# AlexIoannides/bodywork-mlops-demo

Hardware: NVIDIA H100
Metric: train rows/sec (N x 128 least-squares fit) (higher is better)
Workload: dtype bf16x2 (hi+lo) MMA operands, f32 accumulate, f64 fold+solve

## Files before the change

### bodywork-mlops-demo_b200/csrc/b2_internal.cuh

```cuda
#pragma once
#include <cuda.h>
#include <cuda_bf16.h>
#include <cuda_runtime.h>
#include <stdint.h>
#include <stdio.h>
#include <string.h>

#include <type_traits>

#include "../../include/b2gram.h"

namespace b2 {

constexpr int kMaxD = B2_MAX_D;
constexpr int kMaxS = kMaxD + 2;
constexpr int kKernelEventPairs = 64;
constexpr int kMaxRanks = 8;
constexpr size_t kXchgSlotDoubles = (size_t)kMaxS * kMaxS;
constexpr size_t kXchgDataDoubles = 2 * kMaxRanks * kXchgSlotDoubles;
constexpr size_t kXchgBytes = kXchgDataDoubles * sizeof(double) + 256;

constexpr int kTcRows = 64;
constexpr int kTcM = 128;
constexpr int kTcEMax = 16;
// ... 15 lines not shown
constexpr int kRfB0 = kMaxD;
constexpr int kRfMean = kMaxD + 1;
constexpr int kRfPrevBeta = 2 * kMaxD + 1;
constexpr int kRfPrevB0 = 3 * kMaxD + 1;
constexpr int kRfStep = 3 * kMaxD + 2;
constexpr int kRfGrad = 3 * kMaxD + 3;
constexpr int kRfDoubles = kRfGrad + kGradOut;
constexpr int kOutRefineStep = 2 * kMaxD + 3;
constexpr int kOutRefineGuard = 2 * kMaxD + 4;

constexpr int kMaxAlphas = B2_MAX_ALPHAS;
constexpr int kLooQ = 0;
constexpr int kLooLam = kMaxD * kMaxD;
constexpr int kLooMean = kLooLam + kMaxD;
constexpr int kLooC = kLooMean + kMaxD;
constexpr int kLooMisc = kLooC + kMaxD;
constexpr int kLooAlpha = kLooMisc + 8;
constexpr int kLooCw = kLooAlpha + kMaxAlphas;
constexpr int kLooW = kLooCw + kMaxD * kMaxAlphas;
constexpr int kLooSum = kLooW + kMaxD * kMaxAlphas;
constexpr int kLooDoubles = kLooSum + kMaxAlphas;

struct EnetArgs {
  double l1_ratio, eps, tol;
  int n_alphas, grid, max_iter, positive, fit_intercept;
  double* alphas;
  const double* coef_init;
  double *coefs, *intercepts, *gaps, *iters, *tol_out;
  const double* folds = nullptr;
  const double* l1_ratios = nullptr;
  int n_folds = 1, n_l1 = 1;
  double* mse = nullptr;
};

constexpr int kByCoef = 0;
constexpr int kByMisc = kMaxD;
constexpr int kByLambda = kMaxD + 8;
constexpr int kBySigma = 2 * kMaxD + 8;
constexpr int kByDoubles = kBySigma + kMaxD * kMaxD;
constexpr int kStdSigma = 0;
constexpr int kStdMean = kMaxD * kMaxD;
constexpr int kStdCoef = kStdMean + kMaxD;
constexpr int kStdMisc = kStdCoef + kMaxD;
constexpr int kStdDoubles = kStdMisc + 8;
struct BayesArgs {
  double a1, a2, l1, l2, alpha_init, lambda_init;
  double threshold_lambda, tol;
  int max_iter, compute_score, fit_intercept;
  const double* anchor;
  double *out, *scores, *A;
};

constexpr int kGlmSteps = 21;
constexpr int kGlmGrad = 8;
constexpr int kGlmHess = 144;
constexpr int kGlmHp = 144;
constexpr int kGlmPart = kGlmHess + kGlmHp * kGlmHp;
constexpr int kGlmOp = kGlmPart;
constexpr int kGlmOpW = 0, kGlmOpStep = kMaxD, kGlmOpMisc = 2 * kMaxD;
constexpr int kGlmDoubles = kGlmOp + 2 * kMaxD + 8;
enum GlmMode { kGlmGradient = 0, kGlmHessian = 1, kGlmLadder = 2 };
enum GlmFamily { kGlmTweedie = 0, kGlmBinomial = 1 };
constexpr int kGlmCorrect = 7;
enum LabelWord { kLabelKept = 0, kLabelNonFinite, kLabelNonIntegral, kLabelMin, kLabelMax, kLabelNMin, kLabelNMax,
                 kLabelWords };

constexpr int kMaxFolds = 254;
int launch_fold_ranges(b2_ctx* ctx, const uint8_t* fold_of_row, int64_t n, int n_folds, unsigned long long* range);
int launch_fold_sum(b2_ctx* ctx, const double* folds, int n_folds, int d, double* S);

inline int narrow_dp(int d) { return d <= 1 ? 1 : d <= 2 ? 2 : d <= 4 ? 4 : d <= 8 ? 8 : 16; }

void set_error(const char* fmt, ...);

#define B2_CUDA(call)                                                                      \
  do {                                                                                     \
    cudaError_t e_ = (call);                                                               \
    if (e_ != cudaSuccess) {                                                               \
      b2::set_error("%s failed: %s (%s:%d)", #call, cudaGetErrorString(e_), __FILE__, __LINE__); \
      return B2_E_CUDA;                                                                    \
    }                                                                                      \
  } while (0)

}

struct b2_ctx {
  int device = 0;
  int sm_count = 0;
  size_t hbm_bytes = 0;
  char name[128] = {0};
  cudaStream_t stream = nullptr;
  cudaStream_t copy_stream = nullptr;
  cudaEvent_t ev_t0 = nullptr, ev_t1 = nullptr;
  cudaEvent_t ev_k[b2::kKernelEventPairs][2];
  int k_pairs = 0;
  int64_t launches = 0;

  int kernel_mode = B2_KERNEL_AUTO;
  int drain_rows = 8192;
  int precision = B2_PRECISION_SPLIT;

  int d = 0;
  double* S = nullptr;

  double* tc_part = nullptr;
  double* tc_red = nullptr;
  float* shift = nullptr;
  bool solve_attr_set = false;
  double* solve_host = nullptr;
  struct TmCache {
    const void* X = nullptr; const float* y = nullptr; const uint8_t* mask = nullptr;
    int64_t n = 0, ldx = 0; int d = 0, x_dtype = -1;
    int y_map_2d = 0, m_map_2d = 0;
    alignas(64) unsigned char tmX[128], tmY[128], tmM[128];
  } tm_cache;
  double* simt_part = nullptr;
  int simt_ctas = 0;
  double* score_part = nullptr;
  int score_ctas = 0;
  double* coef_dev = nullptr;
  double* grad_part = nullptr;
  double* refine = nullptr;
  double* loo = nullptr;
  double* loo_part = nullptr;
  double* enet = nullptr;
  size_t enet_doubles = 0;
  double* folds = nullptr;
  size_t folds_doubles = 0;
  int n_folds = 0;
  int folds_d = 0;
  unsigned long long* fold_range = nullptr;
  double* glm = nullptr;
  double* glm_part = nullptr;
  double* coef_host = nullptr;
  cudaEvent_t ev_coef[2] = {nullptr, nullptr};
  int coef_slot = 0;
  long long* synth_count = nullptr;
  double* solve_out = nullptr;
  void* stage_x[2] = {nullptr, nullptr};
  float* stage_y[2] = {nullptr, nullptr};
  uint8_t* stage_m[2] = {nullptr, nullptr};
  size_t stage_bytes_x = 0;
  int64_t stage_rows = 0;
  cudaEvent_t ev_copied[2] = {nullptr, nullptr};
  cudaEvent_t ev_consumed[2] = {nullptr, nullptr};
  bool ev_consumed_valid[2] = {false, false};
  char* row_out[2] = {nullptr, nullptr};
  size_t row_out_bytes = 0;
  void* bounce[2] = {nullptr, nullptr};
  cudaEvent_t ev_bounce[2] = {nullptr, nullptr};
  bool s_zero_pending = false;
  void* comm = nullptr;
  int n_ranks = 1, rank = 0;
  double* xchg = nullptr;
  double* xchg_peer[8] = {nullptr};
  bool p2p_ready = false;
  bool p2p_local = false;
  unsigned int xchg_epoch = 0;
  unsigned long long xchg_timeout_ns = 10000000000ull;
  bool xchg_pending = false;
  unsigned int* xchg_status_host = nullptr;
  unsigned int* tc_sync = nullptr;
  int fused_fits = 0;
  int sm_limit = 0;
  bool sm_limit_auto = false;
};

namespace b2 {

inline double* score_totals(const b2_ctx* ctx) { return ctx->score_part + (size_t)ctx->score_ctas * kNStats; }

template <typename... P, typename... A>
int launch_smem(void (*kernel)(P...), int grid, int threads, uint32_t smem, cudaStream_t stream, A... args) {
  B2_CUDA(cudaFuncSetAttribute(kernel, cudaFuncAttributeMaxDynamicSharedMemorySize, smem));
  kernel<<<grid, threads, smem, stream>>>(args...);
  B2_CUDA(cudaGetLastError());
  return B2_OK;
}
template <int V, int... Vs, typename F>
int with_int(int v, F&& f) {
  if constexpr (sizeof...(Vs) == 0) return f(std::integral_constant<int, V>{});
  else return v == V ? f(std::integral_constant<int, V>{}) : with_int<Vs...>(v, f);
}
template <typename F>
int with_rows(int x_dtype, const void* X, F&& f) {
  if (x_dtype == B2_F32) return f(static_cast<const float*>(X));
  return f(static_cast<const __nv_bfloat16*>(X));
}
template <typename P>
using row_t = std::remove_const_t<std::remove_pointer_t<P>>;

// ... 88 lines not shown
```

### bodywork-mlops-demo_b200/csrc/gram_shift.cu

```cuda
#include <cuda_bf16.h>

#include "b2_internal.cuh"
#include "b2_ptx.cuh"

namespace b2 {
namespace {

constexpr int kShiftBlocks = 64;
constexpr int kShiftStride = kMaxD + 1;
constexpr int kShiftPartOff = kMaxD + 1;
constexpr int kShiftTicketOff = kShiftPartOff + kShiftBlocks * kShiftStride;

__host__ __device__ __forceinline__ int64_t shift_samples(int64_t n) { return n < 2048 ? n : 2048; }

__device__ __forceinline__ float shift_round(float c, bool round_bf16) {
  return round_bf16 ? __bfloat162float(__float2bfloat16_rn(c)) : c;
}
__device__ __noinline__ float shift_value(const float* sp, int j, bool round_bf16) {
  float acc = 0.f;
  int cnt = 0;
#pragma unroll 8
  for (int b = 0; b < kShiftBlocks; ++b) {
    const float p = sp[b * kShiftStride + j];
    if (p == p) { acc += p; ++cnt; }
  }
  return shift_round(cnt > 0 ? acc / (float)cnt : 0.f, round_bf16);
}

constexpr int kShiftCols = 160;
constexpr int kShiftGroups = 4;

template <typename T>
__global__ void __launch_bounds__(kShiftCols * kShiftGroups)
tc_shift_kernel(const T* __restrict__ X, const float* __restrict__ y, int64_t n, int d, int64_t ldx, float* shift) {
  __shared__ float sub[kShiftGroups][kShiftCols];
  __shared__ int subn[kShiftGroups][kShiftCols];
  __shared__ bool last_block;
  __shared__ float part_s[kShiftBlocks * kShiftStride];
  float* sp = shift + kShiftPartOff;
  const int j = threadIdx.x % kShiftCols, g = threadIdx.x / kShiftCols;
  const int64_t samples = shift_samples(n);
  const int64_t stride = n / samples;
  const int64_t per = (samples + kShiftBlocks - 1) / kShiftBlocks;
  const int64_t s0 = blockIdx.x * per;
  const int64_t s1 = (s0 + per < samples) ? s0 + per : samples;
  float acc = 0.f;
  int cnt = 0;
  if (j <= d) {
#pragma unroll 8
    for (int64_t s = s0 + g; s < s1; s += kShiftGroups) {
      const int64_t row = s * stride;
      const float v = (j < d) ? raw_ld_global<T>(X + row * ldx + j) : __ldg(y + row);
      const bool finite = fabsf(v) <= 3.0e38f;
      acc += finite ? v : 0.f;
      cnt += finite ? 1 : 0;
    }
  }
  sub[g][j] = acc;
  subn[g][j] = cnt;
  __syncthreads();
  if (g == 0 && j <= d) {
    const int c = subn[0][j] + subn[1][j] + subn[2][j] + subn[3][j];
    sp[blockIdx.x * kShiftStride + (j == d ? kMaxD : j)] =
        c > 0 ? (((sub[0][j] + sub[1][j]) + sub[2][j]) + sub[3][j]) / (float)c : __int_as_float(0x7fc00000);
    __threadfence();
  }
  __syncthreads();
  unsigned int* ticket = reinterpret_cast<unsigned int*>(shift + kShiftTicketOff);
  if (threadIdx.x == 0) last_block = atomicAdd(ticket, 1u) == gridDim.x - 1;
  __syncthreads();
  if (!last_block) return;
  __threadfence();
  if (j <= d) {
    const int col = j == d ? kMaxD : j;
    float p[kShiftBlocks / kShiftGroups];
#pragma unroll
    for (int i = 0; i < kShiftBlocks / kShiftGroups; ++i) p[i] = __ldcg(sp + (g + kShiftGroups * i) * kShiftStride + col);
#pragma unroll
    for (int i = 0; i < kShiftBlocks / kShiftGroups; ++i) part_s[(g + kShiftGroups * i) * kShiftStride + col] = p[i];
  }
  __syncthreads();
  for (int k = threadIdx.x; k <= kMaxD; k += blockDim.x)
    shift[k] = k == kMaxD ? shift_value(part_s, kMaxD, false) : (k < d ? shift_value(part_s, k, sizeof(T) == 2) : 0.f);
  if (threadIdx.x == 0) *ticket = 0u;
}

}

size_t gram_shift_bytes() { return sizeof(float) * (kShiftTicketOff + 1); }

int launch_gram_shift(b2_ctx* ctx, const void* X, int x_dtype, const float* y, int64_t n, int d, int64_t ldx) {
  if (x_dtype == B2_F32)
    tc_shift_kernel<float><<<kShiftBlocks, kShiftCols * kShiftGroups, 0, ctx->stream>>>(
        static_cast<const float*>(X), y, n, d, ldx, ctx->shift);
  else
    tc_shift_kernel<__nv_bfloat16><<<kShiftBlocks, kShiftCols * kShiftGroups, 0, ctx->stream>>>(
        static_cast<const __nv_bfloat16*>(X), y, n, d, ldx, ctx->shift);
  B2_CUDA(cudaGetLastError());
  ctx->launches += 1;
  return B2_OK;
}

}
```

### bodywork-mlops-demo_b200/csrc/gram_tc.cu

```cuda
#include <cuda_bf16.h>
#include <stdlib.h>

#include "b2_internal.cuh"
#include "b2_ptx.cuh"
#include "b2_shift.cuh"
#include "b2_xchg.cuh"

namespace b2 {
namespace {

constexpr int kConsumerWGs = 2;
constexpr int kXformWarps = 8;
constexpr int kThreads = 128 * (kConsumerWGs + 2);
constexpr int kFirstXformWarp = 4 * kConsumerWGs;
constexpr int kTmaWarp = kFirstXformWarp;
constexpr int kEWarp = kFirstXformWarp + 1;
static_assert(kFirstXformWarp + kXformWarps == kThreads / 32, "warp roles");
constexpr int kProducers = kXformWarps;
constexpr int kConsumerWarps = 4 * kConsumerWGs;
constexpr int kKGroups = kTcRows / 8;
constexpr uint32_t kRawStageBytes = kTcRows * kMaxD * 4;
constexpr uint32_t kOpSBO = 128;
constexpr uint32_t kOpLBO = (16 + 2 + 16) * kOpSBO;
constexpr uint32_t kOpEOff = 16 * kOpSBO;
// ... 263 lines not shown
  const int dp = d + 2;
  const int a = min(idx / dp, idx % dp), b = max(idx / dp, idx % dp);
  auto P = [&](int acc, int i, int j) { return __ldcg(red + tc_part_index(acc, i, j, ew)); };
  auto s1 = [&](int i) {
    double t = 0.0;
    for (int blk = 0; blk < pack; ++blk) {
      const int r = blk * d + i, e = kTcM + 3 * blk;
      t += d2 ? P(0, r, e) + P(1, r, e) : P(0, r, e);
    }
    return t;
  };
  auto sxy = [&](int i) {
    double t = 0.0;
    for (int blk = 0; blk < pack; ++blk) {
      const int r = blk * d + i, e = kTcM + 3 * blk;
      t += d2 ? P(0, r, e + 1) + P(0, r, e + 2) + P(1, r, e + 1) + P(1, r, e + 2) : P(0, r, e + 1) + P(0, r, e + 2);
    }
    return t;
  };
  auto G = [&](int i, int j) {
    double g = 0.0;
    for (int blk = 0; blk < pack; ++blk) {
      const int ia = blk * d + i, ib = blk * d + j;
      const double g1 = P(0, min(ia, ib), max(ia, ib));
      g += d2 ? g1 + P(1, ia, ib) + P(1, ib, ia) : g1;
    }
    return g;
  };
  return unshift_entry(a, b, d, c, G, s1, sxy, __ldcg(red + kTcAccElems + 2), __ldcg(red + kTcAccElems + 0),
                       __ldcg(red + kTcAccElems + 1));
}

template <typename T, int DFIX, bool SPLIT, bool RAWB = false, int EW = 8>
__global__ void __launch_bounds__(kThreads, 1)
gram_tc_kernel(const __grid_constant__ CUtensorMap tmX, const __grid_constant__ CUtensorMap tmY,
               const __grid_constant__ CUtensorMap tmM, int y_map_2d, int has_mask, int keep,
               int64_t n_rows, int d_arg, int pack, int d_orig, const float* __restrict__ shift,
               int chunk_tiles, double* __restrict__ part, uint32_t wait_ns, uint32_t dbg_arg) {
#ifdef B2_DEV_KNOBS
  const uint32_t dbg = dbg_arg;
#else
  constexpr uint32_t dbg = 0u;
  (void)dbg_arg;
#endif
  using G = TcGeo<RAWB>;
  constexpr int kRawStages = G::kRawStages, kOpStages = G::kOpStages;
  constexpr uint32_t kOffRaw = G::kOffRaw, kOffOp = G::kOffOp, kOffY = G::kOffY, kOffMask = G::kOffMask;
  const int d = DFIX ? DFIX : d_arg;
  extern __shared__ uint8_t smem_raw[];
  const uint32_t sbase = (smem_u32(smem_raw) + 1023u) & ~1023u;
  uint8_t* smem = smem_raw + (sbase - smem_u32(smem_raw));
  const int warp = threadIdx.x >> 5;
  const int lane = threadIdx.x & 31;

  const uint32_t bar_raw_full = sbase + G::kOffBar;
  const uint32_t bar_raw_empty = bar_raw_full + 8 * kRawStages;
  const uint32_t bar_op_full = bar_raw_empty + 8 * kRawStages;
  const uint32_t bar_op_empty = bar_op_full + 8 * kOpStages;
  float* shift_s = reinterpret_cast<float*>(smem + G::kOffShift);

  const int64_t total_tiles = (n_rows + kTcRows - 1) / kTcRows;
  const int64_t tile_begin = (int64_t)blockIdx.x * total_tiles / gridDim.x;
  const int64_t tile_end = (int64_t)(blockIdx.x + 1) * total_tiles / gridDim.x;
  const int my_tiles = (int)(tile_end - tile_begin);

  if (threadIdx.x == 0) {
    for (int s = 0; s < kRawStages; ++s) {
      mbar_init(bar_raw_full + 8 * s, 1);
      mbar_init(bar_raw_empty + 8 * s, kProducers + (RAWB ? kConsumerWarps : 0));
    }
    for (int s = 0; s < kOpStages; ++s) {
      mbar_init(bar_op_full + 8 * s, kProducers);
      mbar_init(bar_op_empty + 8 * s, kConsumerWarps);
    }
    asm volatile("fence.mbarrier_init.release.cluster;" ::: "memory");
  }
  if (warp == kTmaWarp && lane == 0) {
    tma_prefetch_desc(&tmX);
    tma_prefetch_desc(&tmY);
    if (has_mask) tma_prefetch_desc(&tmM);
  }
  for (uint32_t o = threadIdx.x * 16; o < kOpStages * kOpStageBytes; o += kThreads * 16)
    *reinterpret_cast<uint4*>(smem + kOffOp + o) = make_uint4(0, 0, 0, 0);
  for (int j = threadIdx.x; j <= kMaxD; j += kThreads)
    shift_s[j] = j == kMaxD ? shift[kMaxD] : (j < pack * d_orig ? shift[j % d_orig] : 0.f);
  fence_proxy_async_smem();
  __syncthreads();

  if (warp < kConsumerWarps) {
    asm volatile("setmaxnreg.inc.sync.aligned.u32 %0;" ::"n"(G::kConsumerRegs));
    auto consume = [&](auto wg_c) {
      constexpr int WG = decltype(wg_c)::value;
      constexpr int kF1 = kTcM - 64 * WG;
      constexpr int kF2 = RAWB ? kF1 : kTcM;
      constexpr int kC1 = 64 * WG;
      constexpr int kR1 = (kF1 + EW) / 2, kR2 = (kF2 + EW) / 2;
      float acc1[kR1], acc2[kR2];
      using H = TcSums<DFIX, SPLIT, RAWB, EW, WG>;
      double* my_part = part + (size_t)blockIdx.x * kTcAccElems;
      double sums[H::kRegs > 0 ? H::kRegs : 1];
      const bool on_chip_off = (dbg & 256u) != 0u;
      auto slab_addr = [&](int s, int ln) {
        return sbase + G::kOffSlab + (uint32_t)(((4 * H::kSlabBase + (warp & 3) * H::kSlab + s) * 32 + ln) * 8);
      };
      auto store = [&](auto n_regs, int dst_acc, int col0, bool add, auto val) {
        const int ln = (int)lane_id(), row0 = 64 * WG + 16 * (warp & 3) + (ln >> 2);
#pragma unroll
        for (int r = 0; r < decltype(n_regs)::value; ++r) {
          const int col = col0 + 8 * (r >> 2) + 2 * (ln & 3) + (r & 1), h = (r >> 1) & 1, i = row0 + 8 * h;
          const bool lower = dst_acc == 0 && col < kTcM && i > col;
          const double v = val(r, col, h);
          const bool on_chip = dst_acc == 0 && r >= H::kFirstSlab;
          if (on_chip && r >= H::kFirstReg) {
            double& s = sums[r - H::kFirstReg];
            s = add ? __dadd_rn(s, v) : v;
          } else if (on_chip) {
            const uint32_t a = slab_addr(r - H::kFirstSlab, ln);
            st_shared_f64_if(a, add ? __dadd_rn(ld_shared_f64(a), v) : v, !on_chip_off);
          }
          put_f64(my_part + tc_part_index(dst_acc, i, col, EW), v, add, !lower && (!on_chip || on_chip_off));
        }
      };
      auto flush = [&]() {
        const int ln = (int)lane_id(), row0 = 64 * WG + 16 * (warp & 3) + (ln >> 2);
#pragma unroll
        for (int r = H::kFirstSlab; r < H::kR1; ++r) {
          const int col = kC1 + 8 * (r >> 2) + 2 * (ln & 3) + (r & 1), i = row0 + 8 * ((r >> 1) & 1);
          const double s = r >= H::kFirstReg ? sums[r - H::kFirstReg] : ld_shared_f64(slab_addr(r - H::kFirstSlab, ln));
          put_f64(my_part + tc_part_index(0, i, col, EW), s, false, !(col < kTcM && i > col) && !on_chip_off);
        }
      };
      auto drain = [&](const auto& acc, int dst_acc, int col0, bool add) {
        constexpr int kR = sizeof(acc) / sizeof(float);
        if constexpr (RAWB) {
          constexpr int kF = 2 * kR - EW;
          const double s1[2] = {(double)__shfl_sync(0xffffffffu, acc[kF / 2], lane & ~3),
                                (double)__shfl_sync(0xffffffffu, acc[kF / 2 + 2], lane & ~3)};
          store(std::integral_constant<int, kR>{}, dst_acc, col0, add, [&](int r, int col, int h) {
            return col < kTcM ? (double)acc[r] - (double)shift_s[col] * s1[h] : (double)acc[r];
          });
        } else {
          store(std::integral_constant<int, kR>{}, dst_acc, col0, add, [&](int r, int, int) { return (double)acc[r]; });
        }
      };
      auto release = [&](int tile) {
        mbar_arrive(bar_op_empty + 8 * (tile % kOpStages));
        if constexpr (RAWB) mbar_arrive(bar_raw_empty + 8 * (tile % kRawStages));
      };
      constexpr uint32_t a_off = (uint32_t)WG * 8 * kOpSBO;
      int os = 0, held = -1, in_chunk = 0;
      uint32_t oph = 0;
      bool first_chunk = true;
      for (int it = 0; it < my_tiles; ++it) {
        mbar_wait(bar_op_full + 8 * os, oph, wait_ns);
        const uint32_t op_addr = sbase + kOffOp + os * kOpStageBytes;
        wgmma_fence();
#pragma unroll
        for (int k2 = 0; k2 < kTcRows / 16; ++k2) {
          const uint32_t k_addr = op_addr + k2 * 2 * kOpLBO;
          const uint64_t hi_desc = make_smem_desc(k_addr + a_off), lo_desc = make_smem_desc(k_addr + kOpLoOff + a_off);
          const uint32_t sc1 = (in_chunk > 0 || k2 > 0) ? 1u : 0u, sc2 = (it > 0 || k2 > 0) ? 1u : 0u;
          if constexpr (RAWB) {
            const uint64_t x_desc = make_raw_desc(sbase + kOffRaw + (uint32_t)(it % kRawStages) * kRawStageBytes +
                                                  (uint32_t)WG * kRawBoxBytes + k2 * 16 * 128);
            const uint64_t e_desc = make_smem_desc(k_addr + kOpEOff);
            if (!(dbg & 2u)) {
// ... 103 lines not shown
            st_shared_u16(dst + (3 * bl + 2) * 16, yl);
            if (RAWB && has_mask && !use) {
              const uint32_t row = raw_addr + (uint32_t)rr * 128;
              const uint32_t z[4] = {0u, 0u, 0u, 0u};
#pragma unroll
              for (int q = 0; q < 8; ++q) { st_shared_v4(row + 16 * q, z); st_shared_v4(row + kRawBoxBytes + 16 * q, z); }
            }
            a += yv;
            b = fmaf(yv, yv, b);
            c += use ? 1.f : 0.f;
          }
        }
        const uint32_t es = esum();
        st_shared_f64(es, ld_shared_f64(es) + (double)a);
        st_shared_f64(es + 256, ld_shared_f64(es + 256) + (double)b);
        st_shared_f64(es + 512, ld_shared_f64(es + 512) + (double)c);
      }
      if (i < d && !(dbg & 128u)) {
        float c_i[2];
        ld_vals_vec<float, 2>(sbase + G::kOffShift + 4 * (uint32_t)i, c_i);
        for (int g = t / nb; g < kKGroups; g += kXformWarps / nb) {
          const int r0 = g * 8;
          float v0[8], v1[8];
          const uint32_t src = raw_addr + (uint32_t)r0 * ((uint32_t)d * sizeof(T)) + (uint32_t)i * sizeof(T);
#pragma unroll
          for (int k = 0; k < 8; ++k) {
            const uint32_t a = RAWB ? raw_addr + (uint32_t)(i >> 6) * kRawBoxBytes + (uint32_t)(r0 + k) * 128 +
                                          ((((uint32_t)(i & 63) >> 3) ^ (uint32_t)k) << 4) + (uint32_t)(i & 7) * 2
                                    : src + (uint32_t)k * ((uint32_t)d * sizeof(T));
            float x[2];
            if (dbg & 8u) { x[0] = __uint_as_float(src + k); x[1] = __uint_as_float(src - k); }
            else ld_vals_vec<T, 2>(a, x);
            v0[k] = x[0] - c_i[0];
            v1[k] = x[1] - c_i[1];
          }
          if (!full_tile) {
            const int blk = i / d_orig;
#pragma unroll
            for (int k = 0; k < 8; ++k) {
              bool use = (r0 + k) < rows_valid;
              if (use && has_mask) use = (ld_shared_u8(m_addr + (r0 + k) * pack + blk) == (uint32_t)keep);
              if (!use) { v0[k] = 0.f; v1[k] = 0.f; }
            }
          }
          uint32_t h0[4], l0[4], h1[4], l1[4];
#pragma unroll
          for (int p = 0; p < 4; ++p) {
            if constexpr (SPLIT) {
              split2(v0[2 * p], v0[2 * p + 1], h0[p], l0[p]);
              split2(v1[2 * p], v1[2 * p + 1], h1[p], l1[p]);
            } else {
              const __nv_bfloat162 e0 = __floats2bfloat162_rn(v0[2 * p], v0[2 * p + 1]);
              const __nv_bfloat162 e1 = __floats2bfloat162_rn(v1[2 * p], v1[2 * p + 1]);
              h0[p] = *reinterpret_cast<const uint32_t*>(&e0);
              h1[p] = *reinterpret_cast<const uint32_t*>(&e1);
              l0[p] = l1[p] = 0u;
            }
          }
          if (!(dbg & 4u)) {
            const uint32_t dst = op_addr + (uint32_t)g * kOpLBO + st_off;
            uint32_t f[4], s[4];
#pragma unroll
            for (int p = 0; p < 4; ++p) { f[p] = swp ? h1[p] : h0[p]; s[p] = swp ? h0[p] : h1[p]; }
            st_shared_v4(dst + 16 * swp, f);
            st_shared_v4(dst + 16 - 16 * swp, s);
            if constexpr (SPLIT) {
#pragma unroll
              for (int p = 0; p < 4; ++p) { f[p] = swp ? l1[p] : l0[p]; s[p] = swp ? l0[p] : l1[p]; }
              st_shared_v4(dst + kOpLoOff + 16 * swp, f);
              st_shared_v4(dst + kOpLoOff + 16 - 16 * swp, s);
            }
          }
        }
      }
      if (!(dbg & 32u)) fence_proxy_async_smem();
      __syncwarp();
      if (lane == 0) {
        mbar_arrive(bar_op_full + 8 * os);
        mbar_arrive(bar_raw_empty + 8 * rs);
      }
      if (++rs == kRawStages) { rs = 0; rph ^= 1; }
      if (++os == kOpStages) { os = 0; oph ^= 1; }
    }
    if (warp == kEWarp) {
      const uint32_t es = esum();
      double sy = ld_shared_f64(es), syy = ld_shared_f64(es + 256), cnt = ld_shared_f64(es + 512);
#pragma unroll
      for (int o = 16; o > 0; o >>= 1) {
        sy += __shfl_xor_sync(0xffffffffu, sy, o);
        syy += __shfl_xor_sync(0xffffffffu, syy, o);
        cnt += __shfl_xor_sync(0xffffffffu, cnt, o);
      }
      if (lane == 0) {
        double* ys = part + (size_t)gridDim.x * kTcAccElems + kTcSums * blockIdx.x;
        ys[0] = sy; ys[1] = syy; ys[2] = cnt;
      }
    }
  }
}

struct TcFinal {
  int assign;
  int n_ranks, rank;
  unsigned int epoch;
  PeerPtrs peers;
};

constexpr int kFinalizeThreads = 1024;
constexpr int kFinalizeCtas = (kRedElems + kFinalizeThreads / 4 - 1) / (kFinalizeThreads / 4);

__global__ void __launch_bounds__(kFinalizeThreads, 1)
tc_finalize_kernel(const double* part, int n_ctas, double* red, const float* __restrict__ shift, int d, int pack,
                   int ew, int d2, double* S, unsigned int* sync, const TcFinal fin) {
  __shared__ double quarter[kFinalizeThreads];
  __shared__ double c_s[kMaxD + 1];
  for (int j = threadIdx.x; j <= kMaxD; j += blockDim.x) c_s[j] = (double)shift[j];
  {
    constexpr int epb = kFinalizeThreads / 4;
    const int n_acc = tc_part_elems(ew, d2 != 0);
    const int n_red = n_acc + kTcSums;
    const int per = (((n_red + (int)gridDim.x - 1) / (int)gridDim.x) + epb - 1) / epb * epb;
    const int e0 = (int)blockIdx.x * per;
    const int e1 = e0 + per < n_red ? e0 + per : n_red;
    if (e0 < n_red) tc_reduce_range(part, n_ctas, n_acc, red, e0, e1, quarter);
  }
  grid_barrier(sync + 0);
  {
    const int dp = d + 2;
    const int total = dp * dp;
    const size_t slot = xchg_slot_offset(fin.epoch, fin.rank);
    for (int idx = (int)(blockIdx.x * blockDim.x + threadIdx.x); idx < total; idx += (int)(gridDim.x * blockDim.x)) {
      const double val = tc_fold_value(red, c_s, d, pack, ew, d2 != 0, idx);
      const double sv = fin.assign ? val : S[idx] + val;
      S[idx] = sv;
      if (fin.n_ranks > 1) xchg_store_all(fin.peers, fin.n_ranks, slot, idx, sv);
    }
    if (fin.n_ranks > 1) __threadfence_system();
  }
  __syncthreads();
  __shared__ bool last_cta;
  if (threadIdx.x == 0) {
    __threadfence();
    last_cta = (atomicAdd(sync + 2, 1u) == gridDim.x - 1);
    if (last_cta) {
      sync[0] = 0u; sync[2] = 0u;
      __threadfence();
    }
  }
  __syncthreads();
  if (last_cta && fin.n_ranks > 1) xchg_publish(fin.peers, fin.n_ranks, fin.rank, fin.epoch);
}

typedef CUresult (*PFN_encodeTiled)(CUtensorMap*, CUtensorMapDataType, cuuint32_t, void*, const cuuint64_t*,
                                    const cuuint64_t*, const cuuint32_t*, const cuuint32_t*, CUtensorMapInterleave,
                                    CUtensorMapSwizzle, CUtensorMapL2promotion, CUtensorMapFloatOOBfill);

PFN_encodeTiled get_encode() {
  static PFN_encodeTiled fn = nullptr;
  if (fn == nullptr) {
    void* p = nullptr;
    cudaDriverEntryPointQueryResult q;
    if (cudaGetDriverEntryPoint("cuTensorMapEncodeTiled", &p, cudaEnableDefault, &q) == cudaSuccess &&
        q == cudaDriverEntryPointSuccess)
      fn = reinterpret_cast<PFN_encodeTiled>(p);
  }
  return fn;
}

}

bool gram_tc_supported(const void* X, int x_dtype, const float* y, int64_t n, int d, int64_t ldx,
                       const uint8_t* mask) {
  const int es = x_dtype == B2_F32 ? 4 : 2;
  if (d < 4 || d > kMaxD) return false;
  if ((d * es) % 16 != 0) return false;
  if ((ldx * es) % 16 != 0) return false;
  if ((reinterpret_cast<uintptr_t>(X) & 15) != 0 || (reinterpret_cast<uintptr_t>(y) & 15) != 0) return false;
  if (mask != nullptr && (reinterpret_cast<uintptr_t>(mask) & 15) != 0) return false;
  if (n < kTcRows) return false;
  if (n > (int64_t)0x7fffffff) return false;
  return true;
}

static int encode_vec(PFN_encodeTiled encode, CUtensorMap* tm, CUtensorMapDataType type, int es, const void* v,
                      int64_t n, cuuint32_t box, int* view_2d, const char* what) {
  const cuuint32_t estr[2] = {1, 1};
  const cuuint64_t dims[1] = {(cuuint64_t)n}, strides[1] = {0};
  CUresult r = CUDA_ERROR_INVALID_VALUE;
  if (box <= 256)
    r = encode(tm, type, 1, const_cast<void*>(v), dims, strides, &box, estr, CU_TENSOR_MAP_INTERLEAVE_NONE,
               CU_TENSOR_MAP_SWIZZLE_NONE, CU_TENSOR_MAP_L2_PROMOTION_NONE, CU_TENSOR_MAP_FLOAT_OOB_FILL_NONE);
  *view_2d = r != CUDA_SUCCESS;
  const int k = 16 / es;
  if (r != CUDA_SUCCESS && n % k == 0) {
    const cuuint64_t dims2[2] = {(cuuint64_t)k, (cuuint64_t)(n / k)}, strides2[1] = {16};
    const cuuint32_t box2[2] = {(cuuint32_t)k, box / k};
    r = encode(tm, type, 2, const_cast<void*>(v), dims2, strides2, box2, estr, CU_TENSOR_MAP_INTERLEAVE_NONE,
               CU_TENSOR_MAP_SWIZZLE_NONE, CU_TENSOR_MAP_L2_PROMOTION_NONE, CU_TENSOR_MAP_FLOAT_OOB_FILL_NONE);
// ... 23 lines not shown
                        CU_TENSOR_MAP_FLOAT_OOB_FILL_NONE);
    if (r != CUDA_SUCCESS) {
      set_error("cuTensorMapEncodeTiled(X) failed with %d (n=%lld d=%d box=%d ldx=%lld)", (int)r, (long long)n, d, d_box,
                (long long)ldx);
      return B2_E_CUDA;
    }
  }
  if (int r = encode_vec(encode, tmY_out, CU_TENSOR_MAP_DATA_TYPE_FLOAT32, 4, y, n_y, y_box, y_map_2d_out, "y")) return r;
  if (mask == nullptr) return B2_OK;
  return encode_vec(encode, tmM_out, CU_TENSOR_MAP_DATA_TYPE_UINT8, 1, mask, n_y, y_box, m_map_2d_out, "mask");
}

int64_t gram_tc_main_rows(int64_t n_in, int d_in, int64_t ldx_in, int* pack_out) {
  int pack = 1;
  if (d_in > 16 && d_in <= 64 && ldx_in == d_in) {
    pack = 128 / d_in;
    if (pack > kMaxPack) pack = kMaxPack;
    if (n_in < (int64_t)2 * kTcRows * pack) pack = 1;
  }
  const int group = pack == 1 ? 1 : (pack == 3 ? 48 : (pack == 5 ? 80 : 16));
  if (pack_out != nullptr) *pack_out = pack;
  return n_in - n_in % group;
}

int launch_gram_tc(b2_ctx* ctx, const void* X, int x_dtype, const float* y, int64_t n_in, int d_in, int64_t ldx_in,
                   const uint8_t* mask, int keep, bool assign, unsigned int scatter_epoch) {
  PFN_encodeTiled encode = get_encode();
  if (encode == nullptr) {
    set_error("cuTensorMapEncodeTiled is not available from the driver");
    return B2_E_CUDA;
  }
  const int es = x_dtype == B2_F32 ? 4 : 2;
  int pack = 1;
  const int64_t n_main = gram_tc_main_rows(n_in, d_in, ldx_in, &pack);
  const int64_t n = n_main / pack;
  const int d = pack > 1 ? 128 : d_in;
  const int d_tensor = d_in * pack;
  const int64_t ldx = ldx_in * pack;
  const int64_t n_y = n_main;
  const bool rawb = x_dtype == B2_BF16 && d_in == 128 && pack == 1;
  CUtensorMap tmX, tmY, tmM;
  b2_ctx::TmCache& tc = ctx->tm_cache;
  const bool cached = tc.X == X && tc.y == y && tc.mask == mask && tc.n == n_in && tc.ldx == ldx_in && tc.d == d_in &&
                      tc.x_dtype == x_dtype;
  if (cached) {
    memcpy(&tmX, tc.tmX, sizeof(tmX)); memcpy(&tmY, tc.tmY, sizeof(tmY)); memcpy(&tmM, tc.tmM, sizeof(tmM));
  } else {
    int y_map_2d = 0, m_map_2d = 0;
    if (int r = encode_maps(encode, X, x_dtype, es, y, n, d_tensor, d, ldx, n_y, pack, mask, rawb, &tmX, &tmY, &tmM, &y_map_2d,
                            &m_map_2d))
      return r;
    tc.X = X; tc.y = y; tc.mask = mask; tc.n = n_in; tc.ldx = ldx_in; tc.d = d_in; tc.x_dtype = x_dtype;
    tc.y_map_2d = y_map_2d; tc.m_map_2d = m_map_2d;
    memcpy(tc.tmX, &tmX, sizeof(tmX)); memcpy(tc.tmY, &tmY, sizeof(tmY)); memcpy(tc.tmM, &tmM, sizeof(tmM));
  }

  const int64_t total_tiles = (n + kTcRows - 1) / kTcRows;
  const int sms = (ctx->sm_limit > 0 && ctx->sm_limit < ctx->sm_count) ? ctx->sm_limit : ctx->sm_count;
  const int grid = (int)(total_tiles < sms ? total_tiles : sms);
  int chunk_tiles = ctx->drain_rows / kTcRows / (rawb ? 4 : 1);
  if (chunk_tiles < 1) chunk_tiles = 1;

#ifdef B2_DEV_KNOBS
  static const uint32_t wait_ns = []() {
    const char* e = getenv("B2_WAIT_HINT_NS");
    return e ? (uint32_t)atoi(e) : 20000u;
  }();
#else
  constexpr uint32_t wait_ns = 20000u;
#endif
#ifdef B2_DEV_KNOBS
  static const uint32_t dbg = []() {
    const char* e = getenv("B2_TC_DEBUG");
    return e ? (uint32_t)atoi(e) : 0u;
  }();
#else
  constexpr uint32_t dbg = 0u;
#endif
  const bool split = ctx->precision == B2_PRECISION_SPLIT;
  const int ew = tc_e_width(pack);
  const bool d2 = split && !rawb;
  decltype(&gram_tc_kernel<float, 0, false>) kernel = nullptr;
  uint32_t smem = TcGeo<false>::kSmemBytes;
  with_rows(x_dtype, X, [&](auto* Xr) {
    using T = row_t<decltype(Xr)>;
    return with_int<0, 1>(split, [&](auto SP) {
      constexpr bool kSplit = decltype(SP)::value;
      if (d != 128) kernel = gram_tc_kernel<T, 0, kSplit>;
      else if (ew == 16) kernel = gram_tc_kernel<T, 128, kSplit, false, 16>;
      else kernel = gram_tc_kernel<T, 128, kSplit>;
      if constexpr (std::is_same_v<T, __nv_bfloat16>) {
        if (rawb) {
          kernel = gram_tc_kernel<T, 128, kSplit, true>;
          smem = TcGeo<true>::kSmemBytes;
        }
      }
      return B2_OK;
    });
  });
  B2_CUDA(cudaFuncSetAttribute(kernel, cudaFuncAttributeMaxDynamicSharedMemorySize, smem));
  const int pair = ctx->k_pairs % kKernelEventPairs;
  B2_CUDA(cudaEventRecord(ctx->ev_k[pair][0], ctx->stream));
  kernel<<<grid, kThreads, smem, ctx->stream>>>(tmX, tmY, tmM, tc.y_map_2d, mask != nullptr ? 1 + tc.m_map_2d : 0, keep,
                                                n, d, pack, d_in, ctx->shift, chunk_tiles, ctx->tc_part, wait_ns, dbg);
  B2_CUDA(cudaGetLastError());
  B2_CUDA(cudaEventRecord(ctx->ev_k[pair][1], ctx->stream));
  ctx->k_pairs += 1;

  TcFinal fin;
  memset(&fin, 0, sizeof(fin));
  fin.assign = assign ? 1 : 0;
  fin.n_ranks = 1;
  if (scatter_epoch != 0) {
    fin.n_ranks = ctx->n_ranks; fin.rank = ctx->rank; fin.epoch = scatter_epoch;
    for (int r = 0; r < kMaxRanks; ++r) fin.peers.p[r] = ctx->xchg_peer[r];
  }
  {
    cudaLaunchConfig_t cfg;
    memset(&cfg, 0, sizeof(cfg));
    cfg.gridDim = dim3(kFinalizeCtas < sms ? kFinalizeCtas : sms);
    cfg.blockDim = dim3(kFinalizeThreads); cfg.dynamicSmemBytes = 0; cfg.stream = ctx->stream;
    cudaLaunchAttribute attr[1];
    attr[0].id = cudaLaunchAttributeCooperative;
    attr[0].val.cooperative = 1;
    cfg.attrs = attr; cfg.numAttrs = 1;
    const double* part_arg = ctx->tc_part;
    const float* shift_arg = ctx->shift;
    B2_CUDA(cudaLaunchKernelEx(&cfg, tc_finalize_kernel, part_arg, grid, ctx->tc_red, shift_arg, d_in, pack, ew,
                               d2 ? 1 : 0, ctx->S, ctx->tc_sync, fin));
  }
  ctx->launches += 2;
  return B2_OK;
}

}
```

### bodywork-mlops-demo_b200/csrc/solve.cu

```cuda
#include "b2_internal.cuh"
#include "b2_xchg.cuh"

namespace b2 {
namespace {

constexpr int kOutIntercept = kMaxD;
constexpr int kOutInfo = kMaxD + 1;
constexpr int kOutRank = kMaxD + 2;
constexpr int kOutSingular = kMaxD + 3;
constexpr int kOutRows = kOutSingular + kMaxD;

struct LdcgStat {
  const double* S;
  __device__ __forceinline__ double operator()(int i) const { return __ldcg(S + i); }
};

template <class Stat>
__device__ void build_normal_equations_of(const Stat& S, int d, double alpha, int fit_intercept,
                                       double* A, double* r, double* mean, double* ybar_out) {
  const int dp = d + 2, pitch = d + 1;
  const double n = S(d * dp + d);
  const double inv_n = n > 0.0 ? 1.0 / n : 0.0;
  double sxy = 0.0;
  if ((int)threadIdx.x < d) {
    const double sx = S(threadIdx.x * dp + d);
    sxy = S(threadIdx.x * dp + d + 1);
    mean[threadIdx.x] = fit_intercept ? sx * inv_n : 0.0;
  }
  const double ybar = fit_intercept ? S(d * dp + d + 1) * inv_n : 0.0;
  __syncthreads();
  if ((int)threadIdx.x < d) r[threadIdx.x] = sxy - n * mean[threadIdx.x] * ybar;
  const int lane = threadIdx.x & 31, warp = threadIdx.x >> 5, nwarps = blockDim.x >> 5;
  for (int i0 = warp; i0 < d; i0 += 2 * nwarps) {
    const int i1 = i0 + nwarps;
    double v[8];
#pragma unroll
    for (int u = 0; u < 4; ++u) {
      const int j = lane + 32 * u;
      v[u] = j < d ? S(i0 * dp + j) : 0.0;
      v[4 + u] = (j < d && i1 < d) ? S(i1 * dp + j) : 0.0;
    }
    const double m0 = mean[i0], m1 = i1 < d ? mean[i1] : 0.0;
#pragma unroll
    for (int u = 0; u < 4; ++u) {
      const int j = lane + 32 * u;
      if (j < d) {
        const double mj = mean[j];
        A[i0 * pitch + j] = v[u] - n * m0 * mj + (i0 == j ? alpha : 0.0);
        if (i1 < d) A[i1 * pitch + j] = v[4 + u] - n * m1 * mj + (i1 == j ? alpha : 0.0);
      }
    }
  }
  if (threadIdx.x == 0) *ybar_out = ybar;
  __syncthreads();
}

__device__ __forceinline__ void build_normal_equations(const double* S, int d, double alpha, int fit_intercept,
                                                       double* A, double* r, double* mean, double* ybar_out) {
  build_normal_equations_of(LdcgStat{S}, d, alpha, fit_intercept, A, r, mean, ybar_out);
}

__device__ __forceinline__ double rcp_pos(double x) {
  double y;
  asm("rcp.approx.ftz.f64 %0, %1;" : "=d"(y) : "d"(x));
  const double er = fma(-x, y, 1.0);
  const double t = fma(er, er, er);
  return fma(y, t, y);
}

struct SolveXchg {
  double* own;
  int n_ranks;
  unsigned int epoch;
  unsigned long long timeout_ns;
};

constexpr int kNB = 16;
constexpr int kCholThreads = 512;
constexpr int kUPitch = kNB + 1;

__device__ void refine_update(const double* S, int d, int fit_intercept, bool singular, const double* dbeta, double* misc,
                              double* __restrict__ rf, double* __restrict__ out);

template <bool REFINE>
__global__ void __launch_bounds__(kCholThreads, 1)
solve_cholesky_kernel(double* S, int d, double alpha, int fit_intercept, double* __restrict__ out, const SolveXchg xc,
                      double* __restrict__ rf) {
  extern __shared__ double sm[];
  const int pitch = d + 1;
  double* A = sm;
  double* r = A + d * pitch;
  double* mean = A + (d + 1) * pitch;
  double* invd = mean + d;
  double* misc = invd + d;
  double* U = misc + 8;
  const int tid = threadIdx.x, lane = tid & 31;
  const int warp = __shfl_sync(0xffffffffu, tid >> 5, 0);
  long long tm[5] = {0, 0, 0, 0, 0};
  long long tc0 = clock64();
  if (xc.own != nullptr) {
    __shared__ int ok;
    if (tid == 0) ok = xchg_wait(xc.own, xc.n_ranks, xc.epoch, xc.timeout_ns) ? 1 : 0;
    __syncthreads();
    if (!ok) {
      if (tid == 0) {
        xchg_flags(xc.own)[kXchgStatusWord] = xc.epoch;
        out[kOutInfo] = -1.0;
      }
      return;
    }
    const int dp = d + 2;
    for (int base = 0; base < dp * dp; base += 4 * blockDim.x) {
      double sv[4];
#pragma unroll
      for (int u = 0; u < 4; ++u) {
        const int idx = base + u * blockDim.x + tid;
        sv[u] = idx < dp * dp ? xchg_sum(xc.own, xc.n_ranks, xc.epoch, idx) : 0.0;
      }
#pragma unroll
      for (int u = 0; u < 4; ++u) {
        const int idx = base + u * blockDim.x + tid;
        if (idx < dp * dp) S[idx] = sv[u];
      }
    }
    __threadfence();
    __syncthreads();
  }
  build_normal_equations(S, d, alpha, fit_intercept, A, r, mean, &misc[0]);
  if constexpr (REFINE) {
    if (tid < d) r[tid] = rf[kRfGrad + tid] - alpha * rf[kRfBeta + tid];
    __syncthreads();
  }
  tm[0] = clock64() - tc0;
  if (warp == 0) {
    double mx = 0.0;
    for (int i = lane; i < d; i += 32) mx = fmax(mx, A[i * pitch + i]);
#pragma unroll
    for (int o = 16; o > 0; o >>= 1) mx = fmax(mx, __shfl_xor_sync(0xffffffffu, mx, o));
    if (lane == 0) { misc[1] = mx; misc[2] = 0.0; }
  }
  __syncthreads();
  const double tiny = misc[1] * 1e-12;
  const int rows = d + 1;

  for (int kb = 0; kb < d; kb += kNB) {
    const int nb = (d - kb) < kNB ? (d - kb) : kNB;
    tc0 = clock64();
    if (warp == 0) {
      const int lrow = lane & (kNB - 1), h = lane >> 4;
      const bool act = lrow < nb;
      const int row = kb + (act ? lrow : 0);
      double a[kNB / 2];
#pragma unroll
      for (int cc = 0; cc < kNB / 2; ++cc) {
        const int c = 2 * cc + h;
        a[cc] = (act && c < nb) ? A[row * pitch + kb + c] : 0.0;
      }
      double my_rc = 1.0;
      int first_bad = 0;
#pragma unroll
      for (int k = 0; k < kNB; ++k) {
        if (k < nb) {
          const int hk = k & 1, kk = k >> 1;
          const double colk = a[kk];
          const double piv = __shfl_sync(0xffffffffu, colk, k | (hk << 4));
          const bool bad = !(piv > tiny);
          const double rc = bad ? 1.0 : rcp_pos(piv);
          const double u = __shfl_sync(0xffffffffu, colk, lrow | (hk << 4));
          my_rc = (lrow == k) ? rc : my_rc;
          first_bad = (bad && first_bad == 0) ? (kb + k + 1) : first_bad;
#pragma unroll
          for (int cc = 0; cc < kNB / 2; ++cc) {
            if (2 * cc + 1 > k) {
              const int c = 2 * cc + h;
              const double uc = __shfl_sync(0xffffffffu, colk, c | (hk << 4));
              if (c > k) a[cc] = fma(-(u * uc), rc, a[cc]);
            }
          }
          if (h == hk && act && lrow > k) {
            A[row * pitch + kb + k] = u * rc;
            U[row * kUPitch + k] = u;
// ... 1308 lines not shown
    if (tid < d && keep[tid] != 0.0) {
      g = 1.0 + lmb[tid] * M[tid * pitch + tid];
      lmb[tid] = (g + 2.0 * a.l1) / (coef[tid] * coef[tid] + 2.0 * a.l2);
    }
    alpha = (n - block_sum(g, red) + 2.0 * a.a1) / (sse + 2.0 * a.a2);
    double kept = 0.0;
    if (tid < d) {
      kept = lmb[tid] < a.threshold_lambda ? 1.0 : 0.0;
      keep[tid] = kept;
      if (kept == 0.0) coef[tid] = 0.0;
    }
    nkeep = block_sum(kept, red);
    if (a.compute_score) {
      double t1 = 0.0, t2 = 0.0, t3 = 0.0;
      if (tid < d) {
        t1 = a.l1 * log(lmb[tid]) - a.l2 * lmb[tid];
        t2 = log(lmb[tid]);
        t3 = lmb[tid] * coef[tid] * coef[tid];
      }
      double s = block_sum(t1, red);
      const double slog = block_sum(t2, red), sq = block_sum(t3, red);
      s += a.a1 * log(alpha) - a.a2 * alpha;
      s += 0.5 * (-ld + n * log(alpha) + slog);
      s -= 0.5 * (alpha * sse + sq);
      if (tid == 0) a.scores[iter] = s;
    }
    if (iter > 0 && block_sum(tid < d ? fabs(coef_old[tid] - coef[tid]) : 0.0, red) < a.tol) break;
    if (tid < d) coef_old[tid] = coef[tid];
    if (nkeep == 0.0) break;
  }
  const int n_iter = iter < a.max_iter ? iter + 1 : a.max_iter;
  if (!singular && nkeep > 0.0 && isnan(solve())) singular = true;
  const double mc = block_sum(tid < d ? mean[tid] * coef[tid] : 0.0, red);
  for (int t = tid; t < d * d; t += blockDim.x) {
    const int i = t / d, j = t - i * d;
    a.out[kBySigma + t] = !singular && nkeep > 0.0 && keep[i] != 0.0 && keep[j] != 0.0 ? -M[i * pitch + j] : 0.0;
  }
  if (tid < d) {
    a.out[kByCoef + tid] = coef[tid];
    a.out[kByLambda + tid] = lmb[tid];
  }
  if (tid == 0) {
    a.out[kByMisc + 0] = a.fit_intercept ? misc[0] - mc : 0.0;
    a.out[kByMisc + 1] = alpha;
    a.out[kByMisc + 3] = n_iter;
    a.out[kByMisc + 4] = misc[1];
  }
}

size_t solve_smem_bytes(int d) {
  const size_t chol = (size_t)(d + 1) * (d + 1) + 3 * d + 16 + (size_t)(d + 1) * kUPitch;
  const size_t eig = (size_t)(d + 1) * (d + 1) + 3 * d + 16 + 4 * kMaxD + kMaxD + 2 * (kMaxD + 8) + kMaxD;
  return sizeof(double) * (chol > eig ? chol : eig);
}

int ensure_solve_attrs(b2_ctx* ctx) {
  if (!ctx->solve_attr_set) {
    const int bytes = (int)solve_smem_bytes(kMaxD);
    B2_CUDA(cudaFuncSetAttribute(solve_cholesky_kernel<false>, cudaFuncAttributeMaxDynamicSharedMemorySize, bytes));
    B2_CUDA(cudaFuncSetAttribute(solve_cholesky_kernel<true>, cudaFuncAttributeMaxDynamicSharedMemorySize, bytes));
    B2_CUDA(cudaFuncSetAttribute(solve_spectral_kernel, cudaFuncAttributeMaxDynamicSharedMemorySize, bytes));
    B2_CUDA(cudaFuncSetAttribute(solve_eigvals_kernel, cudaFuncAttributeMaxDynamicSharedMemorySize, bytes));
    B2_CUDA(cudaFuncSetAttribute(solve_eigh_kernel, cudaFuncAttributeMaxDynamicSharedMemorySize,
                                 (int)eigh_smem_bytes(kMaxD)));
    B2_CUDA(cudaFuncSetAttribute(solve_enet_kernel, cudaFuncAttributeMaxDynamicSharedMemorySize,
                                 (int)enet_smem_bytes(kMaxD)));
    B2_CUDA(cudaFuncSetAttribute(bayes_ridge_kernel, cudaFuncAttributeMaxDynamicSharedMemorySize,
                                 (int)bayes_smem_bytes(kMaxD)));
    B2_CUDA(cudaFuncSetAttribute(ard_kernel, cudaFuncAttributeMaxDynamicSharedMemorySize, (int)ard_smem_bytes(kMaxD)));
    ctx->solve_attr_set = true;
  }
  return B2_OK;
}

}

int launch_solve_cholesky(b2_ctx* ctx, double alpha, int fit_intercept, unsigned int gather_epoch) {
  if (int r = ensure_solve_attrs(ctx)) return r;
  SolveXchg xc;
  xc.own = gather_epoch != 0 ? ctx->xchg : nullptr;
  xc.n_ranks = ctx->n_ranks;
  xc.epoch = gather_epoch;
  xc.timeout_ns = ctx->xchg_timeout_ns;
  solve_cholesky_kernel<false><<<1, kCholThreads, solve_smem_bytes(ctx->d), ctx->stream>>>(ctx->S, ctx->d, alpha,
                                                                                           fit_intercept, ctx->solve_host,
                                                                                           xc, nullptr);
  B2_CUDA(cudaGetLastError());
  ctx->launches += 1;
  return B2_OK;
}

int launch_solve_refine(b2_ctx* ctx, double alpha, int fit_intercept) {
  if (int r = ensure_solve_attrs(ctx)) return r;
  SolveXchg xc;
  xc.own = nullptr;
  xc.n_ranks = 1;
  xc.epoch = 0;
  xc.timeout_ns = 0;
  solve_cholesky_kernel<true><<<1, kCholThreads, solve_smem_bytes(ctx->d), ctx->stream>>>(ctx->S, ctx->d, alpha,
                                                                                          fit_intercept, ctx->solve_host,
                                                                                          xc, ctx->refine);
  B2_CUDA(cudaGetLastError());
  ctx->launches += 1;
  return B2_OK;
}

int launch_solve_spectral(b2_ctx* ctx, double cond, int fit_intercept) {
  if (int r = ensure_solve_attrs(ctx)) return r;
  solve_spectral_kernel<<<1, 512, solve_smem_bytes(ctx->d), ctx->stream>>>(ctx->S, ctx->d, cond, fit_intercept, ctx->solve_out);
  B2_CUDA(cudaGetLastError());
  ctx->launches += 1;
  return B2_OK;
}

int launch_solve_eigh(b2_ctx* ctx, int fit_intercept) {
  if (int r = ensure_solve_attrs(ctx)) return r;
  solve_eigh_kernel<<<1, kEighThreads, eigh_smem_bytes(ctx->d), ctx->stream>>>(ctx->S, ctx->d, fit_intercept, ctx->loo);
  B2_CUDA(cudaGetLastError());
  ctx->launches += 1;
  return B2_OK;
}

int launch_solve_enet(b2_ctx* ctx, const EnetArgs& args) {
  if (int r = ensure_solve_attrs(ctx)) return r;
  const int ctas = args.folds != nullptr ? args.n_folds * args.n_l1 : 1;
  solve_enet_kernel<<<ctas, kEnetThreads, enet_smem_bytes(ctx->d), ctx->stream>>>(ctx->S, ctx->d, args);
  B2_CUDA(cudaGetLastError());
  ctx->launches += 1;
  return B2_OK;
}

int launch_bayes_ridge(b2_ctx* ctx, const BayesArgs& args) {
  if (int r = ensure_solve_attrs(ctx)) return r;
  bayes_ridge_kernel<<<1, kByThreads, bayes_smem_bytes(ctx->d), ctx->stream>>>(ctx->S, ctx->d, ctx->loo, args);
  B2_CUDA(cudaGetLastError());
  ctx->launches += 1;
  return B2_OK;
}

int launch_ard(b2_ctx* ctx, const BayesArgs& args) {
  if (int r = ensure_solve_attrs(ctx)) return r;
  ard_kernel<<<1, kByThreads, ard_smem_bytes(ctx->d), ctx->stream>>>(ctx->S, ctx->d, args);
  B2_CUDA(cudaGetLastError());
  ctx->launches += 1;
  return B2_OK;
}

int launch_solve_eigvals(b2_ctx* ctx, double cond, int fit_intercept) {
  if (int r = ensure_solve_attrs(ctx)) return r;
  solve_eigvals_kernel<<<1, kEigThreads, solve_smem_bytes(ctx->d), ctx->stream>>>(ctx->S, ctx->d, cond, fit_intercept,
                                                                                  ctx->solve_out);
  B2_CUDA(cudaGetLastError());
  ctx->launches += 1;
  return B2_OK;
}

}
```

Baseline: 5.623 billion.

## Chain shift, gram, finalize and solve kernels with programmatic dependent launch

Launches the gram, finalize and Cholesky solve kernels with programmatic stream serialization and adds griddepcontrol wait/launch_dependents calls, so each kernel's prologue (smem zeroing, setup) can overlap the tail of the previous kernel. It also caches the per-variant cudaFuncSetAttribute call in the context so it is not issued on every fit. This aims to cut launch gaps and host overhead in a short chain of kernels. The risk is ordering: data visibility now depends on the wait being placed before any read of prior outputs, and a cooperative launch is combined with the PDL attribute.

```diff
diff --git a/bodywork-mlops-demo_b200/csrc/b2_internal.cuh b/bodywork-mlops-demo_b200/csrc/b2_internal.cuh
--- a/bodywork-mlops-demo_b200/csrc/b2_internal.cuh
+++ b/bodywork-mlops-demo_b200/csrc/b2_internal.cuh
@@ -121,6 +121,24 @@
     }                                                                                      \
   } while (0)
 
+__device__ __forceinline__ void griddep_wait() { asm volatile("griddepcontrol.wait;" ::: "memory"); }
+__device__ __forceinline__ void griddep_launch_dependents() { asm volatile("griddepcontrol.launch_dependents;" ::: "memory"); }
+
+template <typename... P, typename... A>
+cudaError_t launch_chained(void (*kernel)(P...), dim3 grid, dim3 block, size_t smem, cudaStream_t stream, bool cooperative,
+                           A&&... args) {
+  cudaLaunchConfig_t cfg;
+  memset(&cfg, 0, sizeof(cfg));
+  cfg.gridDim = grid; cfg.blockDim = block; cfg.dynamicSmemBytes = smem; cfg.stream = stream;
+  cudaLaunchAttribute attr[2];
+  attr[0].id = cudaLaunchAttributeProgrammaticStreamSerialization;
+  attr[0].val.programmaticStreamSerializationAllowed = 1;
+  attr[1].id = cudaLaunchAttributeCooperative;
+  attr[1].val.cooperative = 1;
+  cfg.attrs = attr; cfg.numAttrs = cooperative ? 2 : 1;
+  return cudaLaunchKernelEx(&cfg, kernel, static_cast<A&&>(args)...);
+}
+
 }
 
 struct b2_ctx {
@@ -146,6 +164,7 @@
   double* tc_red = nullptr;
   float* shift = nullptr;
   bool solve_attr_set = false;
+  uint32_t gram_attr_set = 0;
   double* solve_host = nullptr;
   struct TmCache {
     const void* X = nullptr; const float* y = nullptr; const uint8_t* mask = nullptr;
diff --git a/bodywork-mlops-demo_b200/csrc/gram_shift.cu b/bodywork-mlops-demo_b200/csrc/gram_shift.cu
--- a/bodywork-mlops-demo_b200/csrc/gram_shift.cu
+++ b/bodywork-mlops-demo_b200/csrc/gram_shift.cu
@@ -37,6 +37,7 @@
   __shared__ int subn[kShiftGroups][kShiftCols];
   __shared__ bool last_block;
   __shared__ float part_s[kShiftBlocks * kShiftStride];
+  griddep_launch_dependents();
   float* sp = shift + kShiftPartOff;
   const int j = threadIdx.x % kShiftCols, g = threadIdx.x / kShiftCols;
   const int64_t samples = shift_samples(n);
diff --git a/bodywork-mlops-demo_b200/csrc/gram_tc.cu b/bodywork-mlops-demo_b200/csrc/gram_tc.cu
--- a/bodywork-mlops-demo_b200/csrc/gram_tc.cu
+++ b/bodywork-mlops-demo_b200/csrc/gram_tc.cu
@@ -369,6 +369,7 @@
   }
   for (uint32_t o = threadIdx.x * 16; o < kOpStages * kOpStageBytes; o += kThreads * 16)
     *reinterpret_cast<uint4*>(smem + kOffOp + o) = make_uint4(0, 0, 0, 0);
+  griddep_wait();
   for (int j = threadIdx.x; j <= kMaxD; j += kThreads)
     shift_s[j] = j == kMaxD ? shift[kMaxD] : (j < pack * d_orig ? shift[j % d_orig] : 0.f);
   fence_proxy_async_smem();
@@ -638,6 +639,7 @@
       if (++rs == kRawStages) { rs = 0; rph ^= 1; }
       if (++os == kOpStages) { os = 0; oph ^= 1; }
     }
+    if (issuer) griddep_launch_dependents();
     if (warp == kEWarp) {
       const uint32_t es = esum();
       double sy = ld_shared_f64(es), syy = ld_shared_f64(es + 256), cnt = ld_shared_f64(es + 512);
@@ -670,6 +672,8 @@
                    int ew, int d2, double* S, unsigned int* sync, const TcFinal fin) {
   __shared__ double quarter[kFinalizeThreads];
   __shared__ double c_s[kMaxD + 1];
+  griddep_wait();
+  griddep_launch_dependents();
   for (int j = threadIdx.x; j <= kMaxD; j += blockDim.x) c_s[j] = (double)shift[j];
   {
     constexpr int epb = kFinalizeThreads / 4;
@@ -859,28 +863,34 @@
   const bool d2 = split && !rawb;
   decltype(&gram_tc_kernel<float, 0, false>) kernel = nullptr;
   uint32_t smem = TcGeo<false>::kSmemBytes;
+  int variant = 0;
   with_rows(x_dtype, X, [&](auto* Xr) {
     using T = row_t<decltype(Xr)>;
     return with_int<0, 1>(split, [&](auto SP) {
       constexpr bool kSplit = decltype(SP)::value;
       if (d != 128) kernel = gram_tc_kernel<T, 0, kSplit>;
-      else if (ew == 16) kernel = gram_tc_kernel<T, 128, kSplit, false, 16>;
-      else kernel = gram_tc_kernel<T, 128, kSplit>;
+      else if (ew == 16) { kernel = gram_tc_kernel<T, 128, kSplit, false, 16>; variant = 1; }
+      else { kernel = gram_tc_kernel<T, 128, kSplit>; variant = 2; }
       if constexpr (std::is_same_v<T, __nv_bfloat16>) {
         if (rawb) {
           kernel = gram_tc_kernel<T, 128, kSplit, true>;
           smem = TcGeo<true>::kSmemBytes;
+          variant = 3;
         }
       }
       return B2_OK;
     });
   });
-  B2_CUDA(cudaFuncSetAttribute(kernel, cudaFuncAttributeMaxDynamicSharedMemorySize, smem));
+  const uint32_t instance = 1u << (variant + 4 * (split ? 1 : 0) + 8 * (x_dtype == B2_F32 ? 0 : 1));
+  if (!(ctx->gram_attr_set & instance)) {
+    B2_CUDA(cudaFuncSetAttribute(kernel, cudaFuncAttributeMaxDynamicSharedMemorySize, smem));
+    ctx->gram_attr_set |= instance;
+  }
   const int pair = ctx->k_pairs % kKernelEventPairs;
   B2_CUDA(cudaEventRecord(ctx->ev_k[pair][0], ctx->stream));
-  kernel<<<grid, kThreads, smem, ctx->stream>>>(tmX, tmY, tmM, tc.y_map_2d, mask != nullptr ? 1 + tc.m_map_2d : 0, keep,
-                                                n, d, pack, d_in, ctx->shift, chunk_tiles, ctx->tc_part, wait_ns, dbg);
-  B2_CUDA(cudaGetLastError());
+  B2_CUDA(launch_chained(kernel, dim3(grid), dim3(kThreads), smem, ctx->stream, false, tmX, tmY, tmM, tc.y_map_2d,
+                         mask != nullptr ? 1 + tc.m_map_2d : 0, keep, n, d, pack, d_in, (const float*)ctx->shift,
+                         chunk_tiles, ctx->tc_part, wait_ns, dbg));
   B2_CUDA(cudaEventRecord(ctx->ev_k[pair][1], ctx->stream));
   ctx->k_pairs += 1;
 
@@ -892,20 +902,9 @@
     fin.n_ranks = ctx->n_ranks; fin.rank = ctx->rank; fin.epoch = scatter_epoch;
     for (int r = 0; r < kMaxRanks; ++r) fin.peers.p[r] = ctx->xchg_peer[r];
   }
-  {
-    cudaLaunchConfig_t cfg;
-    memset(&cfg, 0, sizeof(cfg));
-    cfg.gridDim = dim3(kFinalizeCtas < sms ? kFinalizeCtas : sms);
-    cfg.blockDim = dim3(kFinalizeThreads); cfg.dynamicSmemBytes = 0; cfg.stream = ctx->stream;
-    cudaLaunchAttribute attr[1];
-    attr[0].id = cudaLaunchAttributeCooperative;
-    attr[0].val.cooperative = 1;
-    cfg.attrs = attr; cfg.numAttrs = 1;
-    const double* part_arg = ctx->tc_part;
-    const float* shift_arg = ctx->shift;
-    B2_CUDA(cudaLaunchKernelEx(&cfg, tc_finalize_kernel, part_arg, grid, ctx->tc_red, shift_arg, d_in, pack, ew,
-                               d2 ? 1 : 0, ctx->S, ctx->tc_sync, fin));
-  }
+  B2_CUDA(launch_chained(tc_finalize_kernel, dim3(kFinalizeCtas < sms ? kFinalizeCtas : sms), dim3(kFinalizeThreads), 0,
+                         ctx->stream, true, (const double*)ctx->tc_part, grid, ctx->tc_red, (const float*)ctx->shift, d_in,
+                         pack, ew, d2 ? 1 : 0, ctx->S, ctx->tc_sync, fin));
   ctx->launches += 2;
   return B2_OK;
 }
diff --git a/bodywork-mlops-demo_b200/csrc/solve.cu b/bodywork-mlops-demo_b200/csrc/solve.cu
--- a/bodywork-mlops-demo_b200/csrc/solve.cu
+++ b/bodywork-mlops-demo_b200/csrc/solve.cu
@@ -97,6 +97,7 @@
   const int tid = threadIdx.x, lane = tid & 31;
   const int warp = __shfl_sync(0xffffffffu, tid >> 5, 0);
   long long tm[5] = {0, 0, 0, 0, 0};
+  griddep_wait();
   long long tc0 = clock64();
   if (xc.own != nullptr) {
     __shared__ int ok;
@@ -1571,10 +1572,8 @@
   xc.n_ranks = ctx->n_ranks;
   xc.epoch = gather_epoch;
   xc.timeout_ns = ctx->xchg_timeout_ns;
-  solve_cholesky_kernel<false><<<1, kCholThreads, solve_smem_bytes(ctx->d), ctx->stream>>>(ctx->S, ctx->d, alpha,
-                                                                                           fit_intercept, ctx->solve_host,
-                                                                                           xc, nullptr);
-  B2_CUDA(cudaGetLastError());
+  B2_CUDA(launch_chained(solve_cholesky_kernel<false>, dim3(1), dim3(kCholThreads), solve_smem_bytes(ctx->d), ctx->stream,
+                         false, ctx->S, ctx->d, alpha, fit_intercept, ctx->solve_host, xc, (double*)nullptr));
   ctx->launches += 1;
   return B2_OK;
 }
@@ -1586,10 +1585,8 @@
   xc.n_ranks = 1;
   xc.epoch = 0;
   xc.timeout_ns = 0;
-  solve_cholesky_kernel<true><<<1, kCholThreads, solve_smem_bytes(ctx->d), ctx->stream>>>(ctx->S, ctx->d, alpha,
-                                                                                          fit_intercept, ctx->solve_host,
-                                                                                          xc, ctx->refine);
-  B2_CUDA(cudaGetLastError());
+  B2_CUDA(launch_chained(solve_cholesky_kernel<true>, dim3(1), dim3(kCholThreads), solve_smem_bytes(ctx->d), ctx->stream,
+                         false, ctx->S, ctx->d, alpha, fit_intercept, ctx->solve_host, xc, ctx->refine));
   ctx->launches += 1;
   return B2_OK;
 }
```

Result: no change. 5.687 billion, median of 6 (+1.1%).
